# Zain-Jiang/Speech-Editing-Toolkit

Measured on AMD Instinct MI355X. Metric: diffusion mel-frames/s (100-step p_sample, B=32/GPU, T=800), higher is better.
Workload: dtype f32 (operands carried as 2 fp16 pieces, 3 MFMA products per term, fp32 accumulate: fp32-equivalent, see roofline.note)

## Files before the change

### speech-editing-toolkit_amd/csrc/diffnet_x3.hip

```cpp
#include <stdio.h>
#include <stdlib.h>

#include "common.h"

#ifndef SET_X3_EXP
#define SET_X3_EXP 0
#endif

typedef __bf16 bf16x8_t __attribute__((ext_vector_type(8)));
typedef unsigned u32x4_t __attribute__((ext_vector_type(4)));
typedef unsigned u32x2_t __attribute__((ext_vector_type(2)));

__device__ uint64_t *g_x3_phase_buf = nullptr;
#ifndef SET_X3_PROBE
#define SET_X3_PROBE 0
#endif

namespace {

constexpr int XC = 256;
constexpr int X_MAXD = 8;
constexpr int XR = XC * 2 + 16;
constexpr int X_KS1 = 48;
constexpr int X_KS2 = 16;
// ... 413 lines not shown
                for (int r = 0; r < 16; ++r)
                    buf_store_agent((acc[u][0][cb][r] * is2) * RSQRT2, rxo, vo4[cb], (unsigned)(row0(u, 0) + urow(r)) * T4);
        }
    }
    const bool first = a.first != 0;
    if constexpr (NU != 1) {
        if (!first) load_sk();
    }
#pragma unroll
    for (int cb = 0; cb < NCB; ++cb) {
        if (tv[cb]) {
            const rsrc_t rsk = make_rsrc(a.skp + ub[cb]);
#pragma unroll
            for (int u = 0; u < NU; ++u)
#pragma unroll
                for (int r = 0; r < 16; ++r)
                    buf_store_agent(first ? acc[u][1][cb][r] * is2 : acc[u][1][cb][r] * is2 + sk[u][cb][r], rsk, vo4[cb],
                                    (unsigned)(32 * (NU * w + u) + urow(r)) * T4);
        }
    }
}
#undef X3_PHASE

template <typename S, int NU, int NCB>
__global__ void __launch_bounds__(512 / NU, NU) diffnet_stack_x3_kernel(SetDiffnetStackArgs a, int tiles_per_utt, int ntiles, int ntasks,
                                                                        unsigned piece_bytes, int fault_tile) {
    extern __shared__ __attribute__((aligned(16))) unsigned char lds[];
    int *s_task = reinterpret_cast<int *>(lds + S::NP * piece_bytes + NCB * XC * sizeof(float));
    int *counter = a.sync_ws, *abort_flag = a.sync_ws + 1, *done = a.sync_ws + 4;
    const int tid = threadIdx.x;
    uint64_t *dbg = (SET_X3_PROBE && blockIdx.x == 0 && tid == 0) ? g_x3_phase_buf : nullptr;
    uint64_t tprev = dbg ? __builtin_amdgcn_s_memtime() : 0;
    if (tid == 0) s_task[0] = atomicAdd(counter, 1);
    __syncthreads();
    int n = __builtin_amdgcn_readfirstlane(s_task[0]);
    int i_done = -1, l_done = 0;
    while (n < ntasks) {
        const int l = n / ntiles, i = n - l * ntiles, j = i;
        X3Tile lt;
        lt.xin = (l & 1) ? a.xb : a.xa;
        lt.xout = (l & 1) ? a.xa : a.xb;
        lt.skp = a.skip;
        lt.cp = a.condproj + (int64_t)l * a.cp_ls; lt.cp_bs = a.cp_bs;
        lt.dstep = a.dstep + (int64_t)l * a.d_ls; lt.d_bs = a.d_bs; lt.d_cs = a.d_cs;
        lt.img = reinterpret_cast<const unsigned short *>(a.wx3_all) + (int64_t)l * x_nimg<S>();
        lt.b_dil = a.b_dil_all + (int64_t)l * 512;
        lt.b_out = a.b_out_all + (int64_t)l * 512;
        lt.err_flag = a.err_flag;
        lt.T = a.T; lt.dil = 1 << (l % a.dilation_cycle_length); lt.first = (l == 0);
        lt.nbu = (a.T + 31) / 32; lt.Q = a.B * lt.nbu; lt.q0 = i * NCB;
        f32x16 acc[NU][2][NCB];
        if constexpr (NU == 1) x3_init<NU, NCB>(lt, acc);
        __builtin_amdgcn_sched_barrier(0);
        const int *f0 = done + i, *fl = done + (j > 0 ? i - 1 : i), *fr = done + (j < tiles_per_utt - 1 ? i + 1 : i);
        int peek = l, claimed = 0;
        if (tid == 0) {
            if (l > 0) peek = min(ld_agent(f0), min(ld_agent(fl), ld_agent(fr)));
            claimed = atomicAdd(counter, 1);
        }
        if (dbg) { const uint64_t tn = __builtin_amdgcn_s_memtime(); dbg[11] += tn - tprev; tprev = tn; }
        asm volatile("s_waitcnt vmcnt(0)" ::: "memory");
        if (dbg) { const uint64_t tn = __builtin_amdgcn_s_memtime(); dbg[12] += tn - tprev; tprev = tn; }
        if (tid == 0) {
            if (peek >= l) __builtin_amdgcn_fence(__ATOMIC_ACQUIRE, "agent");
            s_task[0] = claimed;
            s_task[1] = peek >= l ? 1 : 2;
        }
        __syncthreads();
        if (tid == 0 && i_done >= 0 && !(l_done == 0 && i_done == fault_tile))
            __hip_atomic_store(done + i_done, l_done + 1, __ATOMIC_RELAXED, __HIP_MEMORY_SCOPE_AGENT);
        i_done = -1;
        if (__builtin_amdgcn_readfirstlane(s_task[1]) == 2) {
            if (tid == 0) {
                int ok = 1;
                unsigned spins = 0;
                for (;;) {
                    const int v0 = ld_agent(f0), v1 = ld_agent(fl), v2 = ld_agent(fr);
                    if (min(v0, min(v1, v2)) >= l) break;
                    __builtin_amdgcn_s_sleep(8);
                    if (++spins > X_SPIN_LIMIT || ld_agent(abort_flag) != 0) {
                        __hip_atomic_store(abort_flag, 1, __ATOMIC_RELAXED, __HIP_MEMORY_SCOPE_AGENT);
                        if (a.err_flag) __hip_atomic_store(a.err_flag, 1, __ATOMIC_RELAXED, __HIP_MEMORY_SCOPE_AGENT);
                        ok = 0;
                        break;
                    }
                }
                __builtin_amdgcn_fence(__ATOMIC_ACQUIRE, "agent");
                s_task[2] = ok;
            }
            __syncthreads();
            if (__builtin_amdgcn_readfirstlane(s_task[2]) == 0) break;
        }
        const int n_next = __builtin_amdgcn_readfirstlane(s_task[0]);
        x3_main<S, NU, NCB>(lt, acc, lds, piece_bytes, dbg, tprev);
        i_done = i;
        l_done = l;
        n = n_next;
        if (dbg) {
            const uint64_t tn = __builtin_amdgcn_s_memtime();
            dbg[5] += tn - tprev;
            dbg[7] += 1;
            tprev = tn;
        }
    }
    asm volatile("s_waitcnt vmcnt(0)" ::: "memory");
    __syncthreads();
    if (tid == 0 && i_done >= 0 && !(l_done == 0 && i_done == fault_tile))
        __hip_atomic_store(done + i_done, l_done + 1, __ATOMIC_RELAXED, __HIP_MEMORY_SCOPE_AGENT);
}

template <typename S, int NU, int NCB>
int launch_x3(const SetDiffnetStackArgs &a, int n_cu, int fault_tile, hipStream_t s) {
    static bool attr_set = false;
    if (!attr_set) {
        SET_HIP(hipFuncSetAttribute(reinterpret_cast<const void *>(diffnet_stack_x3_kernel<S, NU, NCB>),
                                    hipFuncAttributeMaxDynamicSharedMemorySize, 160 * 1024), "set_diffnet_stack(x3 attr)");
        attr_set = true;
    }
    const int Q = a.B * ((a.T + 31) / 32);
    const int ntiles = (Q + NCB - 1) / NCB, tiles_per_utt = ntiles;
    const int64_t ntasks64 = (int64_t)ntiles * a.L;
    SET_REQUIRE(ntasks64 < (1ll << 30), "set_diffnet_stack(task count)");
    SET_REQUIRE((int64_t)2 * XC * a.T * 4 < ((int64_t)1 << 31), "set_diffnet_stack(split-operand kernel: T too large)");
    const int max_dil = 1 << (a.dilation_cycle_length - 1);
    const unsigned piece_bytes = (unsigned)(NCB * (32 + 2 * max_dil) * XR);
    const size_t ldsz = x3_lds_bytes<S, NCB>(max_dil);
    SET_HIP(set_zero_async(a.sync_ws, (size_t)(4 + ntiles) * sizeof(int32_t), s), "set_diffnet_stack(memset)");
    int grid = NU * n_cu;
    if (grid > ntiles * 4 / 5) grid = ntiles * 4 / 5;
    if (const char *e = getenv("SET_AMD_STACK_GRID")) grid = atoi(e) > 0 ? atoi(e) : grid;
    if ((int64_t)grid > ntasks64) grid = (int)ntasks64;
    if (grid < 1) grid = 1;
    hipLaunchKernelGGL((diffnet_stack_x3_kernel<S, NU, NCB>), dim3(grid), dim3(512 / NU), ldsz, s, a, tiles_per_utt, ntiles, (int)ntasks64,
                       piece_bytes, fault_tile);
    return set_check_launch("set_diffnet_stack");
}

typedef unsigned u32x2w_t __attribute__((ext_vector_type(2)));
typedef float f32x2 __attribute__((ext_vector_type(2)));
__device__ __forceinline__ f32x2 buf_load2(rsrc_t r, unsigned voff, unsigned soff) {
    return __builtin_bit_cast(f32x2, __builtin_amdgcn_raw_buffer_load_b64(r, (int)voff, (int)soff, 0));
}
__device__ __forceinline__ f32x2 buf_load2_nt(rsrc_t r, unsigned voff, unsigned soff) {
    return __builtin_bit_cast(f32x2, __builtin_amdgcn_raw_buffer_load_b64(r, (int)voff, (int)soff, SET_X3W_NT ? 2 : 0));
}

#ifndef SET_X3V_XRV
#define SET_X3V_XRV (XC * 2 + 32)
#endif
constexpr int XRV = SET_X3V_XRV;
template <int NB> constexpr unsigned xv_piece() { return 16 * NB * XRV; }
template <int NB> constexpr unsigned xv_plane() { return 2 * xv_piece<NB>(); }
template <int NB> constexpr unsigned xv_zpiece() { return 32 * NB * XR; }
template <int NB> constexpr unsigned xv_tile() { return 2 * xv_plane<NB>() > 2 * xv_zpiece<NB>() ? 2 * xv_plane<NB>() : 2 * xv_zpiece<NB>(); }
#ifndef SET_X3V_PF
#define SET_X3V_PF 2
#endif
#ifndef SET_X3V_PF2
#define SET_X3V_PF2 2
#endif
#ifndef SET_X3V_WAVE_PUBLISH
#define SET_X3V_WAVE_PUBLISH 1
#endif
#define X3V_FLAG_UNIT (SET_X3V_WAVE_PUBLISH ? 8 : 1)
#ifndef X3V_LEAD
#define X3V_LEAD 0
#endif
#ifndef SET_X3V_GATE2
#define SET_X3V_GATE2 1
#endif
#ifndef SET_X3V_SLEEP
#define SET_X3V_SLEEP 0
#endif
#ifndef SET_X3V_SLEEP2
#define SET_X3V_SLEEP2 0
#endif
#ifndef SET_X3V_SK_EARLY
#define SET_X3V_SK_EARLY 0
#endif

__device__ __forceinline__ f32x4 mma16(u32x4_t a, u32x4_t b, f32x4 c) {
    return __builtin_amdgcn_mfma_f32_16x16x32_f16(__builtin_bit_cast(f16x8_t, a), __builtin_bit_cast(f16x8_t, b), c, 0, 0, 0);
}
__device__ __forceinline__ float row_prev(float v) {
    return __builtin_bit_cast(float, __builtin_amdgcn_update_dpp(0, __builtin_bit_cast(int, v), 0x111, 0xf, 0xf, false));
}
__device__ __forceinline__ float row_next(float v) {
    return __builtin_bit_cast(float, __builtin_amdgcn_update_dpp(0, __builtin_bit_cast(int, v), 0x101, 0xf, 0xf, false));
}

template <int NB>
__device__ __forceinline__ void x3v_init(const X3Tile &a, f32x4 (&PQ)[2][4][NB]) {
    typedef SplitF16x2 S;
    int tid = threadIdx.x;
    asm volatile("" : "+v"(tid));
    const int lane = tid & 63;
    const int w = __builtin_amdgcn_readfirstlane(tid >> 6);
    const int l15 = lane & 15, kg = lane >> 4;
    const int T = a.T;
    const unsigned T4 = 4u * (unsigned)T;
    const float hs = 0.5f * reinterpret_cast<const float *>(a.img + x_nimg<S>() - 8)[0];
    f32x4 bias[4];
#pragma unroll
    for (int mb = 0; mb < 4; ++mb) bias[mb] = *reinterpret_cast<const f32x4 *>(a.b_dil + (mb >= 2 ? XC : 0) + 32 * w + 16 * (mb & 1) + 4 * kg);
#pragma unroll
    for (int nb = 0; nb < NB; ++nb) {
        const X3Col c = x3_col(a, nb);
        const rsrc_t rcp = make_rsrc(a.cp + (int64_t)c.b * a.cp_bs);
        const unsigned vo = 4u * (unsigned)(4 * kg * T + min(c.t0 + 2 * l15, T - 2));
#pragma unroll
        for (int mb = 0; mb < 4; ++mb) {
            const unsigned row0 = (unsigned)((mb >= 2 ? XC : 0) + 32 * w + 16 * (mb & 1));
#pragma unroll
            for (int i = 0; i < 4; ++i) {
                const f32x2 v = buf_load2_nt(rcp, vo, (row0 + (unsigned)i) * T4);
                const float e = bias[mb][i] + v[0], o = bias[mb][i] + v[1];
                PQ[0][mb][nb][i] = hs * (e + o);
                PQ[1][mb][nb][i] = hs * (e - o);
            }
        }
    }
}

template <int NB, int PH>
__device__ __forceinline__ void x3v_stage_load(const X3Tile &a, int w, int lane, f32x2 (&x12)[NB][8], float (&xh)[NB][8]) {
    const int l15 = lane & 15, cs = lane >> 4;
    const int ch0 = 32 * w + 8 * cs;
    const int T = a.T;
    const unsigned T4 = 4u * (unsigned)T;
    const bool edge = l15 == 0 || l15 == 15;
#pragma unroll
    for (int nb = 0; nb < NB; ++nb) {
        const X3Col c = x3_col(a, nb);
        const rsrc_t rx = make_rsrc(a.xin + (int64_t)c.b * XC * T);
        const int t = c.t0 + 2 * l15;
        const unsigned vox = 4u * (unsigned)min(t, T - 2) + (unsigned)ch0 * T4;
#pragma unroll
        for (int k = 0; k < 8; ++k) x12[nb][k] = buf_load2(rx, vox, (unsigned)k * T4);
        if (PH == 1) {
            const int th = l15 == 0 ? c.t0 - 1 : c.t0 + 32;
            const unsigned voh = 4u * (unsigned)min(max(th, 0), T - 1) + (unsigned)ch0 * T4;
            if (edge) {
#pragma unroll
                for (int k = 0; k < 8; ++k) xh[nb][k] = buf_load(rx, voh, (unsigned)k * T4);
            }
        }
    }
}
template <int NB, int PH>
__device__ __forceinline__ float x3v_stage_store(const X3Tile &a, unsigned char *lds, const float *dsh, int w, int lane, const f32x2 (&x12)[NB][8],
                                                 const float (&xh)[NB][8]) {
    typedef SplitF16x2 S;
    const int l15 = lane & 15, cs = lane >> 4;
    const int ch0 = 32 * w + 8 * cs;
    const int T = a.T;
    const bool edge = l15 == 0 || l15 == 15;
    float amax = 0.0f;
#pragma unroll
    for (int nb = 0; nb < NB; ++nb) {
        const X3Col c = x3_col(a, nb);
        const int t = c.t0 + 2 * l15, th = l15 == 0 ? c.t0 - 1 : c.t0 + 32;
        const bool v12 = c.ok && t < T, vh = c.ok && edge && th >= 0 && th < T;
        const f32x4 dA = *reinterpret_cast<const f32x4 *>(dsh + nb * XC + ch0);
        const f32x4 dB = *reinterpret_cast<const f32x4 *>(dsh + nb * XC + ch0 + 4);
        u32x4_t u[2][2];
#pragma unroll
        for (int e2 = 0; e2 < 4; ++e2) {
            float V[2][2];
#pragma unroll
            for (int h = 0; h < 2; ++h) {
                const int e = 2 * e2 + h;
                const float ds = e < 4 ? dA[e & 3] : dB[e & 3];
                const float d1 = v12 ? x12[nb][e][0] + ds : 0.0f, d2 = v12 ? x12[nb][e][1] + ds : 0.0f;
                if (PH == 0) {
                    V[0][h] = d1 + d2;
                    V[1][h] = d2 - d1;
                } else {
                    float d0 = row_prev(d2), d3 = row_next(d1);
                    const float hv = vh ? xh[nb][e] + ds : 0.0f;
                    d0 = l15 == 0 ? hv : d0;
                    d3 = l15 == 15 ? hv : d3;
                    V[0][h] = d0 - d2;
                    V[1][h] = d1 - d3;
                }
            }
#pragma unroll
            for (int j = 0; j < 2; ++j) {
                amax = fmaxf(fmaxf(amax, fabsf(V[j][0])), fabsf(V[j][1]));
                unsigned pw[2];
                S::split2(V[j][0], V[j][1], pw);
                u[j][0][e2] = pw[0];
                u[j][1][e2] = pw[1];
            }
        }
#pragma unroll
        for (int j = 0; j < 2; ++j)
#pragma unroll
            for (int q = 0; q < 2; ++q) *reinterpret_cast<u32x4_t *>(lds + j * xv_plane<NB>() + q * xv_piece<NB>() + (16 * nb + l15) * XRV + ch0 * 2) = u[j][q];
    }
    return amax;
}

template <int NB, int PFV>
__device__ __forceinline__ void x3v_plane(f32x4 (&acc)[4][NB], u32x4_t (&A)[PFV][4][2], rsrc_t img, unsigned lane16, unsigned abase, int seg,
                                          const unsigned char *bplane, unsigned boff) {
    typedef SplitF16x2 S;
    const int ks_last = 16 * (seg >> 1) + 15;
    for (int kb = 0; kb < 8; kb += PFV) {
#pragma unroll
        for (int p = 0; p < PFV; ++p) {
            const int kc = kb + p, ks = 8 * seg + kc;
            u32x4_t Bv[NB][2];
#pragma unroll
            for (int nb = 0; nb < NB; ++nb)
#pragma unroll
                for (int q = 0; q < 2; ++q) Bv[nb][q] = *reinterpret_cast<const u32x4_t *>(bplane + q * xv_piece<NB>() + boff + (unsigned)(nb * 16 * XRV) + (unsigned)kc * 64u);
            __builtin_amdgcn_sched_barrier(0);
            if (SET_X3V_SLEEP) __builtin_amdgcn_s_sleep(SET_X3V_SLEEP);
            __builtin_amdgcn_s_setprio(1);
#pragma unroll
            for (int t = 0; t < S::NPROD; ++t)
#pragma unroll
                for (int mb = 0; mb < 4; ++mb)
#pragma unroll
                    for (int nb = 0; nb < NB; ++nb) acc[mb][nb] = mma16(A[p][mb][S::qa(t)], Bv[nb][S::qb(t)], acc[mb][nb]);
            __builtin_amdgcn_s_setprio(0);
            const int kn = min(ks + PFV, ks_last);
#pragma unroll
            for (int mb = 0; mb < 4; ++mb)
#pragma unroll
                for (int q = 0; q < 2; ++q) A[p][mb][q] = buf_load_u4(img, lane16, abase + (unsigned)(((kn * 4 + mb) * 2 + q) * 1024));
            __builtin_amdgcn_sched_barrier(0);
        }
    }
}

template <int NB>
__device__ __forceinline__ void x3v_main(const X3Tile &a, f32x4 (&PQ)[2][4][NB], unsigned char *lds, uint64_t *dbg, uint64_t &tprev, uint64_t (&ts)[32]) {
#if SET_X3_PROBE == 2
#define X3V_PHASE(p)                                  \
    {                                                 \
        __builtin_amdgcn_sched_barrier(0);            \
        ts[8 + (p)] = __builtin_amdgcn_s_memtime();   \
        __builtin_amdgcn_sched_barrier(0);            \
    }
#else
#define X3V_PHASE(p)                                          \
    if (dbg) {                                                \
        const uint64_t tn = __builtin_amdgcn_s_memtime();     \
        dbg[p] += tn - tprev;                                 \
        tprev = tn;                                           \
    }
#endif
#if SET_X3_PROBE == 2
#define X3V_TS(p) X3V_PHASE(p)
#else
#define X3V_TS(p)
#endif
    X3V_PHASE(0)
    typedef SplitF16x2 S;
    constexpr int PFV = SET_X3V_PF;
    int tid = threadIdx.x;
    asm volatile("" : "+v"(tid));
    const int lane = tid & 63;
    const int w = __builtin_amdgcn_readfirstlane(tid >> 6);
    const int l15 = lane & 15, kg = lane >> 4;
    const int half = lane >> 5, l31 = lane & 31;
    const int T = a.T;
    const unsigned T4 = 4u * (unsigned)T;
    const unsigned lane16 = 16u * (unsigned)lane;
    float *dsh = reinterpret_cast<float *>(lds + xv_tile<NB>());
    const rsrc_t rw = make_rsrc(a.img);
    const float *sc = reinterpret_cast<const float *>(a.img + x_n1<S>() + x_n2<S>());
    const float s2 = sc[2], is2 = sc[3];
    const float is1w = reinterpret_cast<const float *>(a.img + x_nimg<S>() - 8)[1];
    const float cg2 = is1w * -1.4426950408889634f, cf2 = is1w * 2.8853900817779268f;
    (void)cg2; (void)cf2;
    const unsigned abase = (unsigned)((x_n1<S>() + x_n2<S>() + 8) * 2) + (unsigned)(w * X_KSV * 4 * 2 * 1024);
    const unsigned boff = (unsigned)(l15 * XRV + kg * 16);
    u32x4_t A[PFV][4][2];
    f32x2 x12[NB][8];
    float xh[NB][8];
    x3v_stage_load<NB, 0>(a, w, lane, x12, xh);
    float amax = x3v_stage_store<NB, 0>(a, lds, dsh, w, lane, x12, xh);
#pragma unroll
    for (int p = 0; p < PFV; ++p)
#pragma unroll
        for (int mb = 0; mb < 4; ++mb)
#pragma unroll
            for (int q = 0; q < 2; ++q) A[p][mb][q] = buf_load_u4(rw, lane16, abase + (unsigned)(((p * 4 + mb) * 2 + q) * 1024));
    X3V_TS(12)
    __syncthreads();
    X3V_PHASE(1)
    x3v_plane<NB, PFV>(PQ[0], A, rw, lane16, abase, 0, lds, boff);
    x3v_plane<NB, PFV>(PQ[1], A, rw, lane16, abase, 1, lds + xv_plane<NB>(), boff);
    X3V_PHASE(2)
    x3v_stage_load<NB, 1>(a, w, lane, x12, xh);
    __builtin_amdgcn_sched_barrier(0);
#pragma unroll
    for (int mb = 0; mb < 4; ++mb)
#pragma unroll
        for (int nb = 0; nb < NB; ++nb)
#pragma unroll
            for (int i = 0; i < 4; ++i) {
                const float pp = PQ[0][mb][nb][i], qq = PQ[1][mb][nb][i];
                PQ[0][mb][nb][i] = pp + qq;
                PQ[1][mb][nb][i] = pp - qq;
            }
    __syncthreads();
    X3V_TS(13)
    amax = fmaxf(amax, x3v_stage_store<NB, 1>(a, lds, dsh, w, lane, x12, xh));
    if (!(amax < 32768.0f) && a.err_flag) __hip_atomic_store(a.err_flag, 2, __ATOMIC_RELAXED, __HIP_MEMORY_SCOPE_AGENT);
#pragma unroll
    for (int p = 0; p < PFV; ++p)
#pragma unroll
        for (int mb = 0; mb < 4; ++mb)
#pragma unroll
            for (int q = 0; q < 2; ++q) A[p][mb][q] = buf_load_u4(rw, lane16, abase + (unsigned)((((16 + p) * 4 + mb) * 2 + q) * 1024));
    X3V_TS(14)
    __syncthreads();
    X3V_PHASE(3)
    x3v_plane<NB, PFV>(PQ[0], A, rw, lane16, abase, 2, lds, boff);
    x3v_plane<NB, PFV>(PQ[1], A, rw, lane16, abase, 3, lds + xv_plane<NB>(), boff);
    X3V_PHASE(4)
    bool tv[NB];
    unsigned vo4[NB];
    int64_t ub[NB];
#pragma unroll
    for (int cb = 0; cb < NB; ++cb) {
        const X3Col c = x3_col(a, cb);
        const int t = c.t0 + l31;
        tv[cb] = c.ok && t < T;
        vo4[cb] = 4u * (unsigned)(4 * half * T + min(t, T - 1));
        ub[cb] = (int64_t)c.b * XC * T;
    }
    float xres[NB][16];
#pragma unroll
    for (int cb = 0; cb < NB; ++cb) {
        const rsrc_t rx = make_rsrc(a.xin + ub[cb]);
#pragma unroll
        for (int r = 0; r < 16; ++r) xres[cb][r] = buf_load(rx, vo4[cb], (unsigned)(32 * w + urow(r)) * T4);
    }
    __syncthreads();
    X3V_TS(15)
#pragma unroll
    for (int nb = 0; nb < NB; ++nb) {
        const X3Col c = x3_col(a, nb);
        const bool tvp = c.ok && c.t0 + 2 * l15 < T;
#pragma unroll
        for (int eo = 0; eo < 2; ++eo)
#pragma unroll
            for (int m = 0; m < 2; ++m) {
                float zz[4];
#pragma unroll
                for (int i = 0; i < 4; ++i) {
#if SET_X3V_GATE2
                    const float u = __builtin_amdgcn_exp2f(PQ[eo][m][nb][i] * cg2);
                    const float v = __builtin_amdgcn_exp2f(fminf(PQ[eo][m + 2][nb][i] * cf2, 64.0f));
                    const float g = (v - 1.0f) * __builtin_amdgcn_rcpf((1.0f + u) * (1.0f + v));
#else
                    const float g = fsig(PQ[eo][m][nb][i] * is1w) * ftanh(PQ[eo][m + 2][nb][i] * is1w);
#endif
                    zz[i] = tvp ? g : 0.0f;
                }
                unsigned plo[2], phi[2];
                S::split2(zz[0], zz[1], plo);
                S::split2(zz[2], zz[3], phi);
                const unsigned off = (unsigned)((32 * nb + 2 * l15 + eo) * XR + (32 * w + 16 * m + 4 * kg) * 2);
#pragma unroll
                for (int q = 0; q < 2; ++q) {
                    u32x2w_t uu;
                    uu[0] = plo[q];
                    uu[1] = phi[q];
                    *reinterpret_cast<u32x2w_t *>(lds + q * xv_zpiece<NB>() + off) = uu;
                }
            }
    }
    f32x16 acc[1][2][NB];
#pragma unroll
    for (int rb = 0; rb < 2; ++rb) {
        const float *bo = a.b_out + (rb ? XC : 0) + 32 * w;
#pragma unroll
        for (int r = 0; r < 16; ++r) {
            const float blo = bo[urow(r)], bhi = bo[urow(r) + 4];
            const float bias = half ? bhi : blo;
#pragma unroll
            for (int cb = 0; cb < NB; ++cb) acc[0][rb][cb][r] = (rb == 0 ? bias + xres[cb][r] : bias) * s2;
        }
    }
#if SET_X3V_SK_EARLY
    float sk[NB][16];
#pragma unroll
    for (int cb = 0; cb < NB; ++cb) {
        const rsrc_t rsk = make_rsrc(a.skp + ub[cb]);
#pragma unroll
        for (int r = 0; r < 16; ++r) sk[cb][r] = buf_load_nt(rsk, vo4[cb], (unsigned)(32 * w + urow(r)) * T4);
    }
#endif
    X3V_TS(16)
    __syncthreads();
    X3V_PHASE(8)
    gemm_x3<S, X_KS2, 1, NB, SET_X3V_PF2, SET_X3V_SLEEP2>(acc, rw, lane16, (unsigned)(x_n1<S>() * 2 + w * X_KS2 * 2 * 2 * 1024), (unsigned)(X_KS2 * 2 * 2 * 1024), lds,
                                             xv_zpiece<NB>(), [&](int ks, int cb) { return (unsigned)((cb * 32 + l31) * XR + (ks * 16 + half * 8) * 2); });
    X3V_PHASE(9)
    const bool first = a.first != 0;
#if !SET_X3V_SK_EARLY
    float sk[NB][16];
    if (!first) {
#pragma unroll
        for (int cb = 0; cb < NB; ++cb) {
            const rsrc_t rsk = make_rsrc(a.skp + ub[cb]);
#pragma unroll
            for (int r = 0; r < 16; ++r) sk[cb][r] = buf_load_nt(rsk, vo4[cb], (unsigned)(32 * w + urow(r)) * T4);
        }
    }
#endif
#pragma unroll
    for (int cb = 0; cb < NB; ++cb) {
        if (tv[cb]) {
            const rsrc_t rxo = make_rsrc(a.xout + ub[cb]);
#pragma unroll
            for (int r = 0; r < 16; ++r) buf_store_agent((acc[0][0][cb][r] * is2) * RSQRT2, rxo, vo4[cb], (unsigned)(32 * w + urow(r)) * T4);
        }
    }
    X3V_TS(17)
#pragma unroll
    for (int cb = 0; cb < NB; ++cb) {
        if (tv[cb]) {
            const rsrc_t rsk = make_rsrc(a.skp + ub[cb]);
#pragma unroll
            for (int r = 0; r < 16; ++r)
                buf_store_agent(first ? acc[0][1][cb][r] * is2 : acc[0][1][cb][r] * is2 + sk[cb][r], rsk, vo4[cb], (unsigned)(32 * w + urow(r)) * T4);
        }
    }
    X3V_PHASE(10)
}
#undef X3V_PHASE
#undef X3V_TS

#if SET_X3_PROBE == 2
#ifndef X3V_TL_TASK
#define X3V_TL_TASK 10
#endif
#define X3V_KTS(p)                                \
    {                                             \
        __builtin_amdgcn_sched_barrier(0);        \
        ts[p] = __builtin_amdgcn_s_memtime();     \
        __builtin_amdgcn_sched_barrier(0);        \
    }
#else
#define X3V_KTS(p)
#endif
template <int NB>
__global__ void __launch_bounds__(512, 1) diffnet_stack_x3v_kernel(SetDiffnetStackArgs a, int ntiles, int ntasks, int fault_tile) {
    typedef SplitF16x2 S;
    extern __shared__ __attribute__((aligned(16))) unsigned char lds[];
    int *s_task = reinterpret_cast<int *>(lds + xv_tile<NB>() + NB * XC * sizeof(float));
    int *counter = a.sync_ws, *abort_flag = a.sync_ws + 1, *done = a.sync_ws + 4;
    const int tid = threadIdx.x;
    uint64_t *dbg = (SET_X3_PROBE == 1 && blockIdx.x == 0 && tid == 0) ? g_x3_phase_buf : nullptr;
    uint64_t tprev = dbg ? __builtin_amdgcn_s_memtime() : 0;
    if (tid == 0) s_task[0] = atomicAdd(counter, 1);
    __syncthreads();
    int n = __builtin_amdgcn_readfirstlane(s_task[0]);
    int i_done = -1, l_done = 0;
    uint64_t ts[32] = {};
    int n_mine = 0;
    (void)n_mine;
    while (n < ntasks) {
        const int l = n / ntiles, i = n - l * ntiles;
        X3Tile lt;
        lt.xin = (l & 1) ? a.xb : a.xa;
        lt.xout = (l & 1) ? a.xa : a.xb;
        lt.skp = a.skip;
        lt.cp = a.condproj + (int64_t)l * a.cp_ls; lt.cp_bs = a.cp_bs;
        lt.dstep = a.dstep + (int64_t)l * a.d_ls; lt.d_bs = a.d_bs; lt.d_cs = a.d_cs;
        lt.img = reinterpret_cast<const unsigned short *>(a.wx3_all) + (int64_t)l * x_nimg<S>();
        lt.b_dil = a.b_dil_all + (int64_t)l * 512;
        lt.b_out = a.b_out_all + (int64_t)l * 512;
        lt.err_flag = a.err_flag;
        lt.T = a.T; lt.dil = 1; lt.first = (l == 0);
        lt.nbu = (a.T + 31) / 32; lt.Q = a.B * lt.nbu; lt.q0 = i * NB;
        f32x4 PQ[2][4][NB];
        X3V_KTS(0)
#if SET_X3V_WAVE_PUBLISH
        if (i_done >= 0) {
            asm volatile("s_waitcnt vmcnt(0)" ::: "memory");
            if ((tid & 63) == 0 && !(l_done == 0 && i_done == fault_tile))
                (void)__hip_atomic_fetch_add(done + i_done, 1, __ATOMIC_RELAXED, __HIP_MEMORY_SCOPE_AGENT);
            i_done = -1;
        }
        __builtin_amdgcn_sched_barrier(0);
#endif
        float dsv[(NB * XC + 511) / 512];
#pragma unroll
        for (int j = 0; j < (NB * XC + 511) / 512; ++j) {
            const int idx = min(tid + 512 * j, NB * XC - 1);
            dsv[j] = lt.dstep[(int64_t)x3_col(lt, idx >> 8).b * lt.d_bs + (int64_t)(idx & (XC - 1)) * lt.d_cs];
        }
        x3v_init<NB>(lt, PQ);
        __builtin_amdgcn_sched_barrier(0);
        const int *f0 = done + i, *fl = done + (i > 0 ? i - 1 : i), *fr = done + (i < ntiles - 1 ? i + 1 : i);
        int peek = l, claimed = 0;
        if (tid == X3V_LEAD) {
            if (l > 0) peek = min(ld_agent(f0), min(ld_agent(fl), ld_agent(fr))) / X3V_FLAG_UNIT;
            claimed = atomicAdd(counter, 1);
        }
        X3V_KTS(1)
        asm volatile("s_waitcnt vmcnt(0)" ::: "memory");
        X3V_KTS(2)
        {
            float *dsh = reinterpret_cast<float *>(lds + xv_tile<NB>());
#pragma unroll
            for (int j = 0; j < (NB * XC + 511) / 512; ++j)
                if (tid + 512 * j < NB * XC) dsh[tid + 512 * j] = dsv[j];
        }
        if (tid == X3V_LEAD) {
            if (peek >= l) __builtin_amdgcn_fence(__ATOMIC_ACQUIRE, "agent");
            s_task[0] = claimed;
            s_task[1] = peek >= l ? 1 : 2;
        }
        __syncthreads();
        X3V_KTS(3)
#if !SET_X3V_WAVE_PUBLISH
        if (tid == 0 && i_done >= 0 && !(l_done == 0 && i_done == fault_tile))
            __hip_atomic_store(done + i_done, l_done + 1, __ATOMIC_RELAXED, __HIP_MEMORY_SCOPE_AGENT);
        i_done = -1;
#endif
        if (__builtin_amdgcn_readfirstlane(s_task[1]) == 2) {
            if (tid == X3V_LEAD) {
                int ok = 1;
                unsigned spins = 0;
                for (;;) {
                    const int v0 = ld_agent(f0), v1 = ld_agent(fl), v2 = ld_agent(fr);
                    if (min(v0, min(v1, v2)) >= l * X3V_FLAG_UNIT) break;
                    __builtin_amdgcn_s_sleep(8);
                    if (++spins > X_SPIN_LIMIT || ld_agent(abort_flag) != 0) {
                        __hip_atomic_store(abort_flag, 1, __ATOMIC_RELAXED, __HIP_MEMORY_SCOPE_AGENT);
                        if (a.err_flag) __hip_atomic_store(a.err_flag, 1, __ATOMIC_RELAXED, __HIP_MEMORY_SCOPE_AGENT);
                        ok = 0;
                        break;
                    }
                }
                __builtin_amdgcn_fence(__ATOMIC_ACQUIRE, "agent");
                s_task[2] = ok;
            }
            __syncthreads();
            if (__builtin_amdgcn_readfirstlane(s_task[2]) == 0) break;
        }
        const int n_next = __builtin_amdgcn_readfirstlane(s_task[0]);
        X3V_KTS(4)
        x3v_main<NB>(lt, PQ, lds, dbg, tprev, ts);
#if SET_X3_PROBE == 2
        if (++n_mine == X3V_TL_TASK && (tid == 0 || tid == 448) && g_x3_phase_buf) {
            const rsrc_t rt = make_rsrc(g_x3_phase_buf);
            const unsigned row = (unsigned)(2 * blockIdx.x + (tid ? 1 : 0)) * 128u;
#pragma unroll
            for (int k = 0; k < 32; ++k) __builtin_amdgcn_raw_buffer_store_b32((unsigned)(ts[k] - ts[0]), rt, (int)(row + 4 * k), 0, 0);
            __builtin_amdgcn_raw_buffer_store_b32((unsigned)n, rt, (int)(row + 20), 0, 0);
            __builtin_amdgcn_raw_buffer_store_b32((unsigned)s_task[1], rt, (int)(row + 24), 0, 0);
            __builtin_amdgcn_raw_buffer_store_b32((unsigned)ts[0], rt, (int)(row + 28), 0, 0);
        } else if (n_mine == X3V_TL_TASK + 1 && (tid == 0 || tid == 448) && g_x3_phase_buf) {
            __builtin_amdgcn_raw_buffer_store_b32((unsigned)ts[0], make_rsrc(g_x3_phase_buf), (int)((unsigned)(2 * blockIdx.x + (tid ? 1 : 0)) * 128u + 124u), 0, 0);
        }
#endif
        i_done = i;
        l_done = l;
        n = n_next;
        if (dbg) {
            const uint64_t tn = __builtin_amdgcn_s_memtime();
            dbg[5] += tn - tprev;
            dbg[7] += 1;
            tprev = tn;
        }
    }
    asm volatile("s_waitcnt vmcnt(0)" ::: "memory");
#if SET_X3V_WAVE_PUBLISH
    if ((tid & 63) == 0 && i_done >= 0 && !(l_done == 0 && i_done == fault_tile))
        (void)__hip_atomic_fetch_add(done + i_done, 1, __ATOMIC_RELAXED, __HIP_MEMORY_SCOPE_AGENT);
#else
    __syncthreads();
    if (tid == 0 && i_done >= 0 && !(l_done == 0 && i_done == fault_tile))
        __hip_atomic_store(done + i_done, l_done + 1, __ATOMIC_RELAXED, __HIP_MEMORY_SCOPE_AGENT);
#endif
}

template <int NB>
int launch_x3v(const SetDiffnetStackArgs &a, int n_cu, int fault_tile, hipStream_t s) {
    static bool attr_set = false;
    if (!attr_set) {
        SET_HIP(hipFuncSetAttribute(reinterpret_cast<const void *>(diffnet_stack_x3v_kernel<NB>), hipFuncAttributeMaxDynamicSharedMemorySize, 160 * 1024),
                "set_diffnet_stack(x3v attr)");
        attr_set = true;
    }
    const int Q = a.B * ((a.T + 31) / 32);
    const int ntiles = (Q + NB - 1) / NB;
    const int64_t ntasks64 = (int64_t)ntiles * a.L;
    SET_REQUIRE(ntasks64 < (1ll << 30), "set_diffnet_stack(task count)");
    SET_REQUIRE((int64_t)2 * XC * a.T * 4 < ((int64_t)1 << 31), "set_diffnet_stack(split-operand kernel: T too large)");
    SET_REQUIRE(a.dilation_cycle_length == 1 && a.T % 2 == 0, "set_diffnet_stack(x3v: dilation 1 and even T only)");
    const size_t ldsz = (size_t)xv_tile<NB>() + NB * XC * sizeof(float) + 16;
    SET_HIP(set_zero_async(a.sync_ws, (size_t)(4 + ntiles) * sizeof(int32_t), s), "set_diffnet_stack(memset)");
    int grid = n_cu;
    if (NB == 2 && grid > ntiles * 4 / 5) grid = ntiles * 4 / 5;
    if (const char *e = getenv("SET_AMD_STACK_GRID")) grid = atoi(e) > 0 ? atoi(e) : grid;
    if ((int64_t)grid > ntasks64) grid = (int)ntasks64;
    if (grid < 1) grid = 1;
    hipLaunchKernelGGL(diffnet_stack_x3v_kernel<NB>, dim3(grid), dim3(512), ldsz, s, a, ntiles, (int)ntasks64, fault_tile);
    return set_check_launch("set_diffnet_stack");
}


constexpr unsigned SX_SPIN_LIMIT = 1u << 20;
constexpr int SX_PF = 8;

__device__ __forceinline__ float buf_load_sc1(rsrc_t r, unsigned voff, unsigned soff) {
    return __builtin_bit_cast(float, __builtin_amdgcn_raw_buffer_load_b32(r, (int)voff, (int)soff, 16));
}
__device__ __forceinline__ u32x4_t buf_load_u4_sc1(rsrc_t r, unsigned voff, unsigned soff) {
    return __builtin_amdgcn_raw_buffer_load_b128(r, (int)voff, (int)soff, 16);
}

__device__ __forceinline__ bool sx_wait(const int *f0, const int *f1, const int *f2, int want, int *abort_flag, int *err_flag, bool fence = true) {
    unsigned spins = 0;
    for (;;) {
        const int v0 = ld_agent(f0), v1 = ld_agent(f1), v2 = ld_agent(f2);
        if (min(v0, min(v1, v2)) >= want) break;
        __builtin_amdgcn_s_sleep(1);
        if (++spins > SX_SPIN_LIMIT || ld_agent(abort_flag) != 0) {
            __hip_atomic_store(abort_flag, 1, __ATOMIC_RELAXED, __HIP_MEMORY_SCOPE_AGENT);
            if (err_flag) __hip_atomic_store(err_flag, 1, __ATOMIC_RELAXED, __HIP_MEMORY_SCOPE_AGENT);
            return false;
        }
    }
    if (fence) __builtin_amdgcn_fence(__ATOMIC_ACQUIRE, "agent");
    return true;
}

template <int NKS, typename BF>
__device__ __forceinline__ void sx_gemm(f32x16 &acc, u32x4_t (&A)[SX_PF][2], rsrc_t img, unsigned lane16, unsigned abase,
                                        const unsigned char *lds, unsigned piece_bytes, BF bfrag) {
    unsigned bo = bfrag(0);
    u32x4_t b0 = *reinterpret_cast<const u32x4_t *>(lds + bo);
    u32x4_t b1 = *reinterpret_cast<const u32x4_t *>(lds + piece_bytes + bo);
#pragma unroll 1
    for (int kb = 0; kb < NKS; kb += SX_PF) {
#pragma unroll
        for (int p = 0; p < SX_PF; ++p) {
            const int ks = kb + p;
            const unsigned bn = bfrag(min(ks + 1, NKS - 1));
            const u32x4_t nb0 = *reinterpret_cast<const u32x4_t *>(lds + bn);
            const u32x4_t nb1 = *reinterpret_cast<const u32x4_t *>(lds + piece_bytes + bn);
            acc = SplitF16x2::mma(A[p][1], b0, acc);
            acc = SplitF16x2::mma(A[p][0], b1, acc);
            acc = SplitF16x2::mma(A[p][0], b0, acc);
            const int kn = min(ks + SX_PF, NKS - 1);
            A[p][0] = buf_load_u4(img, lane16, abase + (unsigned)(kn * 4 * 1024));
            A[p][1] = buf_load_u4(img, lane16, abase + (unsigned)((kn * 4 + 1) * 1024));
            b0 = nb0;
            b1 = nb1;
            __builtin_amdgcn_sched_barrier(0);
        }
    }
}
__device__ __forceinline__ void sx_preload(u32x4_t (&A)[SX_PF][2], rsrc_t img, unsigned lane16, unsigned abase) {
#pragma unroll
    for (int p = 0; p < SX_PF; ++p) {
        A[p][0] = buf_load_u4(img, lane16, abase + (unsigned)(p * 4 * 1024));
        A[p][1] = buf_load_u4(img, lane16, abase + (unsigned)((p * 4 + 1) * 1024));
    }
}

__global__ void __launch_bounds__(256, 1) diffnet_stack_split_x2_kernel(SetDiffnetStackArgs a, int tiles_per_utt, int ntiles,
                                                                         unsigned piece_bytes, int fault_tile, int nofence) {
    typedef SplitF16x2 S;
    extern __shared__ __attribute__((aligned(16))) unsigned char lds[];
    float *gs = reinterpret_cast<float *>(lds + 2 * piece_bytes);
    float *dsh = gs + 64 * 32;
    int *s_ok = reinterpret_cast<int *>(dsh + XC);
    int *abort_flag = a.sync_ws + 1, *ready = a.sync_ws + 4, *zcnt = a.sync_ws + 4 + ntiles;
    const int tid = threadIdx.x, lane = tid & 63, half = lane >> 5, l31 = lane & 31;
    const int j = __builtin_amdgcn_readfirstlane(tid >> 6);
    if ((int)blockIdx.x >= 4 * ntiles) {
        const int hp = blockIdx.x & 3;
        for (int l = 1; l < a.L; ++l) {
            unsigned spins = 0;
            while (l >= 2 && ld_agent(ready) < 4 * (l - 1)) {
                __builtin_amdgcn_s_sleep(8);
                if (++spins > SX_SPIN_LIMIT || ld_agent(abort_flag) != 0) return;
            }
            const unsigned char *img = reinterpret_cast<const unsigned char *>(a.wx3_all) + (int64_t)l * x_nimg<S>() * 2;
            const rsrc_t r1 = make_rsrc(img + (size_t)(2 * hp) * X_KS1 * 4 * 1024);
            const rsrc_t r2 = make_rsrc(img + x_n1<S>() * 2 + (size_t)(2 * hp) * X_KS2 * 4 * 1024);
            for (unsigned off = 16u * tid; off < 2u * X_KS1 * 4 * 1024; off += 8u * 4096u) {
#pragma unroll
                for (unsigned q = 0; q < 8; ++q) {
                    const u32x4_t v = buf_load_u4(r1, off + q * 4096u, 0u);
                    asm volatile("" ::"v"(v));
                }
            }
            for (unsigned off = 16u * tid; off < 2u * X_KS2 * 4 * 1024; off += 8u * 4096u) {
#pragma unroll
                for (unsigned q = 0; q < 8; ++q) {
                    const u32x4_t v = buf_load_u4(r2, off + q * 4096u, 0u);
                    asm volatile("" ::"v"(v));
                }
            }
        }
        return;
    }
    const int i = blockIdx.x >> 2, h = blockIdx.x & 3;
    const int b = i / tiles_per_utt, jt = i - b * tiles_per_utt;
    const int T = a.T, t0 = jt * 32;
    const int il = jt > 0 ? i - 1 : i, ir = jt < tiles_per_utt - 1 ? i + 1 : i;
    const unsigned T4 = 4u * (unsigned)T;
    const int w8 = 2 * h + (j & 1), rb = j >> 1;
    const int ch0 = 32 * w8;
    const int tq = t0 + l31;
    const bool tv = tq < T;
    const unsigned vo4 = 4u * (unsigned)(4 * half * T + min(tq, T - 1));
    const unsigned lane16 = 16u * (unsigned)lane;
    unsigned short *zt = reinterpret_cast<unsigned short *>(a.z_ws) + (int64_t)i * (2 * 32 * XC);
    const rsrc_t rz = make_rsrc(zt);
    const rsrc_t rsk = make_rsrc(a.skip + (int64_t)b * XC * T);
    uint64_t *dbg = (SET_X3_PROBE && blockIdx.x == 5 && tid == 0) ? g_x3_phase_buf : nullptr;
    uint64_t tprev = dbg ? __builtin_amdgcn_s_memtime() : 0;
#define SX_PHASE(p)                                           \
    if (dbg) {                                                \
        const uint64_t tn = __builtin_amdgcn_s_memtime();     \
        dbg[p] += tn - tprev;                                 \
        tprev = tn;                                           \
    }
    for (int l = 0; l < a.L; ++l) {
        const int d = 1 << (l % a.dilation_cycle_length);
        const unsigned short *img = reinterpret_cast<const unsigned short *>(a.wx3_all) + (int64_t)l * x_nimg<S>();
        const rsrc_t rw = make_rsrc(img);
        const float *sc = reinterpret_cast<const float *>(img + x_n1<S>() + x_n2<S>());
        const float s1 = sc[0], is1 = sc[1], s2 = sc[2], is2 = sc[3];
        const rsrc_t rxin = make_rsrc(((l & 1) ? a.xb : a.xa) + (int64_t)b * XC * T);
        const rsrc_t rxout = make_rsrc(((l & 1) ? a.xa : a.xb) + (int64_t)b * XC * T);
        const rsrc_t rcp = make_rsrc(a.condproj + (int64_t)l * a.cp_ls + (int64_t)b * a.cp_bs);
        const float *dstep = a.dstep + (int64_t)l * a.d_ls + (int64_t)b * a.d_bs;
        const float *bd = a.b_dil_all + (int64_t)l * 512 + rb * XC + ch0, *bo = a.b_out_all + (int64_t)l * 512 + rb * XC + ch0;
        u32x4_t A[SX_PF][2];
        const unsigned ab1 = (unsigned)(((w8 * X_KS1) * 2 + rb) * 2 * 1024);
        sx_preload(A, rw, lane16, ab1);
        f32x16 acc;
#pragma unroll
        for (int r = 0; r < 16; ++r) {
            const float blo = bd[urow(r)], bhi = bd[urow(r) + 4];
            acc[r] = (half ? bhi : blo) + buf_load(rcp, vo4, (unsigned)(rb * XC + ch0 + urow(r)) * T4);
        }
        if (tid == 0) *s_ok = (l == 0 || sx_wait(ready + i, ready + il, ready + ir, 4 * l, abort_flag, a.err_flag, !nofence)) ? 1 : 0;
        __syncthreads();
// ... 220 lines not shown
```

Measured before the change: 177,800.

## Stage all four x3v operand planes up front using a three-slot LDS layout

The input load, halo load and split of both phases now happen in one pass. Three of the four split planes go to three LDS slots and the fourth stays in registers until slot A is free. This removes the second global load/split stage between the plane GEMMs, and one __syncthreads is placed so that the plane-2 GEMM overlaps the plane-3 store. The cost is more LDS (three planes instead of two) and more live registers, which may reduce occupancy or cause spills.

Measured after the change: 171,300 (median of 6 runs). 3.6% lower.

```diff
diff --git a/speech-editing-toolkit_amd/csrc/diffnet_x3.hip b/speech-editing-toolkit_amd/csrc/diffnet_x3.hip
--- a/speech-editing-toolkit_amd/csrc/diffnet_x3.hip
+++ b/speech-editing-toolkit_amd/csrc/diffnet_x3.hip
@@ -589,7 +589,13 @@
 template <int NB> constexpr unsigned xv_piece() { return 16 * NB * XRV; }
 template <int NB> constexpr unsigned xv_plane() { return 2 * xv_piece<NB>(); }
 template <int NB> constexpr unsigned xv_zpiece() { return 32 * NB * XR; }
-template <int NB> constexpr unsigned xv_tile() { return 2 * xv_plane<NB>() > 2 * xv_zpiece<NB>() ? 2 * xv_plane<NB>() : 2 * xv_zpiece<NB>(); }
+constexpr unsigned x3v_slot_a() { return 0; }
+template <int NB> constexpr unsigned x3v_slot_b() { return xv_plane<NB>(); }
+template <int NB> constexpr unsigned x3v_slot_c() { return 2 * xv_plane<NB>(); }
+template <int NB> constexpr unsigned xv_tile() { return 3 * xv_plane<NB>(); }
+template <int NB> constexpr size_t x3v_lds_bytes() { return (size_t)xv_tile<NB>() + NB * XC * sizeof(float) + 16; }
+static_assert(2 * xv_zpiece<3>() <= x3v_slot_c<3>() && 2 * xv_zpiece<2>() <= x3v_slot_c<2>(), "x3v: the z tile must fit over slots A and B");
+static_assert(x3v_lds_bytes<3>() <= 160 * 1024 && x3v_lds_bytes<2>() <= 160 * 1024, "x3v: LDS layout over the 160 KiB opt-in");
 #ifndef SET_X3V_PF
 #define SET_X3V_PF 2
 #endif
@@ -659,7 +665,7 @@
     }
 }
 
-template <int NB, int PH>
+template <int NB>
 __device__ __forceinline__ void x3v_stage_load(const X3Tile &a, int w, int lane, f32x2 (&x12)[NB][8], float (&xh)[NB][8]) {
     const int l15 = lane & 15, cs = lane >> 4;
     const int ch0 = 32 * w + 8 * cs;
@@ -674,19 +680,17 @@
         const unsigned vox = 4u * (unsigned)min(t, T - 2) + (unsigned)ch0 * T4;
 #pragma unroll
         for (int k = 0; k < 8; ++k) x12[nb][k] = buf_load2(rx, vox, (unsigned)k * T4);
-        if (PH == 1) {
-            const int th = l15 == 0 ? c.t0 - 1 : c.t0 + 32;
-            const unsigned voh = 4u * (unsigned)min(max(th, 0), T - 1) + (unsigned)ch0 * T4;
-            if (edge) {
-#pragma unroll
-                for (int k = 0; k < 8; ++k) xh[nb][k] = buf_load(rx, voh, (unsigned)k * T4);
-            }
-        }
-    }
-}
-template <int NB, int PH>
+        const int th = l15 == 0 ? c.t0 - 1 : c.t0 + 32;
+        const unsigned voh = 4u * (unsigned)min(max(th, 0), T - 1) + (unsigned)ch0 * T4;
+        if (edge) {
+#pragma unroll
+            for (int k = 0; k < 8; ++k) xh[nb][k] = buf_load(rx, voh, (unsigned)k * T4);
+        }
+    }
+}
+template <int NB>
 __device__ __forceinline__ float x3v_stage_store(const X3Tile &a, unsigned char *lds, const float *dsh, int w, int lane, const f32x2 (&x12)[NB][8],
-                                                 const float (&xh)[NB][8]) {
+                                                 const float (&xh)[NB][8], u32x4_t (&u3)[NB][2]) {
     typedef SplitF16x2 S;
     const int l15 = lane & 15, cs = lane >> 4;
     const int ch0 = 32 * w + 8 * cs;
@@ -700,42 +704,53 @@
         const bool v12 = c.ok && t < T, vh = c.ok && edge && th >= 0 && th < T;
         const f32x4 dA = *reinterpret_cast<const f32x4 *>(dsh + nb * XC + ch0);
         const f32x4 dB = *reinterpret_cast<const f32x4 *>(dsh + nb * XC + ch0 + 4);
-        u32x4_t u[2][2];
+        u32x4_t u[3][2];
 #pragma unroll
         for (int e2 = 0; e2 < 4; ++e2) {
-            float V[2][2];
+            float V[4][2];
 #pragma unroll
             for (int h = 0; h < 2; ++h) {
                 const int e = 2 * e2 + h;
                 const float ds = e < 4 ? dA[e & 3] : dB[e & 3];
                 const float d1 = v12 ? x12[nb][e][0] + ds : 0.0f, d2 = v12 ? x12[nb][e][1] + ds : 0.0f;
-                if (PH == 0) {
-                    V[0][h] = d1 + d2;
-                    V[1][h] = d2 - d1;
-                } else {
-                    float d0 = row_prev(d2), d3 = row_next(d1);
-                    const float hv = vh ? xh[nb][e] + ds : 0.0f;
-                    d0 = l15 == 0 ? hv : d0;
-                    d3 = l15 == 15 ? hv : d3;
-                    V[0][h] = d0 - d2;
-                    V[1][h] = d1 - d3;
-                }
-            }
-#pragma unroll
-            for (int j = 0; j < 2; ++j) {
+                float d0 = row_prev(d2), d3 = row_next(d1);
+                const float hv = vh ? xh[nb][e] + ds : 0.0f;
+                d0 = l15 == 0 ? hv : d0;
+                d3 = l15 == 15 ? hv : d3;
+                V[0][h] = d1 + d2;
+                V[1][h] = d2 - d1;
+                V[2][h] = d0 - d2;
+                V[3][h] = d1 - d3;
+            }
+#pragma unroll
+            for (int j = 0; j < 4; ++j) {
                 amax = fmaxf(fmaxf(amax, fabsf(V[j][0])), fabsf(V[j][1]));
                 unsigned pw[2];
                 S::split2(V[j][0], V[j][1], pw);
-                u[j][0][e2] = pw[0];
-                u[j][1][e2] = pw[1];
-            }
-        }
-#pragma unroll
-        for (int j = 0; j < 2; ++j)
+                if (j < 3) {
+                    u[j][0][e2] = pw[0];
+                    u[j][1][e2] = pw[1];
+                } else {
+                    u3[nb][0][e2] = pw[0];
+                    u3[nb][1][e2] = pw[1];
+                }
+            }
+        }
+#pragma unroll
+        for (int j = 0; j < 3; ++j)
 #pragma unroll
             for (int q = 0; q < 2; ++q) *reinterpret_cast<u32x4_t *>(lds + j * xv_plane<NB>() + q * xv_piece<NB>() + (16 * nb + l15) * XRV + ch0 * 2) = u[j][q];
     }
     return amax;
+}
+template <int NB>
+__device__ __forceinline__ void x3v_store_plane3(unsigned char *lds, int w, int lane, const u32x4_t (&u3)[NB][2]) {
+    const int l15 = lane & 15, cs = lane >> 4;
+    const int ch0 = 32 * w + 8 * cs;
+#pragma unroll
+    for (int nb = 0; nb < NB; ++nb)
+#pragma unroll
+        for (int q = 0; q < 2; ++q) *reinterpret_cast<u32x4_t *>(lds + q * xv_piece<NB>() + (16 * nb + l15) * XRV + ch0 * 2) = u3[nb][q];
 }
 
 template <int NB, int PFV>
@@ -816,10 +831,14 @@
     const unsigned abase = (unsigned)((x_n1<S>() + x_n2<S>() + 8) * 2) + (unsigned)(w * X_KSV * 4 * 2 * 1024);
     const unsigned boff = (unsigned)(l15 * XRV + kg * 16);
     u32x4_t A[PFV][4][2];
-    f32x2 x12[NB][8];
-    float xh[NB][8];
-    x3v_stage_load<NB, 0>(a, w, lane, x12, xh);
-    float amax = x3v_stage_store<NB, 0>(a, lds, dsh, w, lane, x12, xh);
+    u32x4_t u3[NB][2];
+    {
+        f32x2 x12[NB][8];
+        float xh[NB][8];
+        x3v_stage_load<NB>(a, w, lane, x12, xh);
+        const float amax = x3v_stage_store<NB>(a, lds, dsh, w, lane, x12, xh, u3);
+        if (!(amax < 32768.0f) && a.err_flag) __hip_atomic_store(a.err_flag, 2, __ATOMIC_RELAXED, __HIP_MEMORY_SCOPE_AGENT);
+    }
 #pragma unroll
     for (int p = 0; p < PFV; ++p)
 #pragma unroll
@@ -829,11 +848,9 @@
     X3V_TS(12)
     __syncthreads();
     X3V_PHASE(1)
-    x3v_plane<NB, PFV>(PQ[0], A, rw, lane16, abase, 0, lds, boff);
-    x3v_plane<NB, PFV>(PQ[1], A, rw, lane16, abase, 1, lds + xv_plane<NB>(), boff);
+    x3v_plane<NB, PFV>(PQ[0], A, rw, lane16, abase, 0, lds + x3v_slot_a(), boff);
+    x3v_plane<NB, PFV>(PQ[1], A, rw, lane16, abase, 1, lds + x3v_slot_b<NB>(), boff);
     X3V_PHASE(2)
-    x3v_stage_load<NB, 1>(a, w, lane, x12, xh);
-    __builtin_amdgcn_sched_barrier(0);
 #pragma unroll
     for (int mb = 0; mb < 4; ++mb)
 #pragma unroll
@@ -844,21 +861,21 @@
                 PQ[0][mb][nb][i] = pp + qq;
                 PQ[1][mb][nb][i] = pp - qq;
             }
+#pragma unroll
+    for (int p = 0; p < PFV; ++p)
+#pragma unroll
+        for (int mb = 0; mb < 4; ++mb)
+#pragma unroll
+            for (int q = 0; q < 2; ++q) A[p][mb][q] = buf_load_u4(rw, lane16, abase + (unsigned)((((16 + p) * 4 + mb) * 2 + q) * 1024));
     __syncthreads();
     X3V_TS(13)
-    amax = fmaxf(amax, x3v_stage_store<NB, 1>(a, lds, dsh, w, lane, x12, xh));
-    if (!(amax < 32768.0f) && a.err_flag) __hip_atomic_store(a.err_flag, 2, __ATOMIC_RELAXED, __HIP_MEMORY_SCOPE_AGENT);
-#pragma unroll
-    for (int p = 0; p < PFV; ++p)
-#pragma unroll
-        for (int mb = 0; mb < 4; ++mb)
-#pragma unroll
-            for (int q = 0; q < 2; ++q) A[p][mb][q] = buf_load_u4(rw, lane16, abase + (unsigned)((((16 + p) * 4 + mb) * 2 + q) * 1024));
+    x3v_store_plane3<NB>(lds + x3v_slot_a(), w, lane, u3);
     X3V_TS(14)
+    x3v_plane<NB, PFV>(PQ[0], A, rw, lane16, abase, 2, lds + x3v_slot_c<NB>(), boff);
+    X3V_PHASE(3)
     __syncthreads();
-    X3V_PHASE(3)
-    x3v_plane<NB, PFV>(PQ[0], A, rw, lane16, abase, 2, lds, boff);
-    x3v_plane<NB, PFV>(PQ[1], A, rw, lane16, abase, 3, lds + xv_plane<NB>(), boff);
+    X3V_TS(18)
+    x3v_plane<NB, PFV>(PQ[1], A, rw, lane16, abase, 3, lds + x3v_slot_a(), boff);
     X3V_PHASE(4)
     bool tv[NB];
     unsigned vo4[NB];
@@ -1136,7 +1153,7 @@
     SET_REQUIRE(ntasks64 < (1ll << 30), "set_diffnet_stack(task count)");
     SET_REQUIRE((int64_t)2 * XC * a.T * 4 < ((int64_t)1 << 31), "set_diffnet_stack(split-operand kernel: T too large)");
     SET_REQUIRE(a.dilation_cycle_length == 1 && a.T % 2 == 0, "set_diffnet_stack(x3v: dilation 1 and even T only)");
-    const size_t ldsz = (size_t)xv_tile<NB>() + NB * XC * sizeof(float) + 16;
+    const size_t ldsz = x3v_lds_bytes<NB>();
     SET_HIP(set_zero_async(a.sync_ws, (size_t)(4 + ntiles) * sizeof(int32_t), s), "set_diffnet_stack(memset)");
     int grid = n_cu;
     if (NB == 2 && grid > ntiles * 4 / 5) grid = ntiles * 4 / 5;
```
